# SolverForge/solverforge

Measured on AMD Instinct MI355X. Metric: moves-evaluated/sec, CVRP-1000 (nearby-list selector, LateAcceptance(400)+AcceptedCount(256)), higher is better.
Workload: dtype int64 score / int32 trial deltas (u16 matrix copy)

## Files before the change

solverforge_amd/_lib.py:

```python
import ctypes as C
import os

import numpy as np

_DIR = os.path.dirname(os.path.abspath(__file__))
LIB_PATH = os.environ.get("SF_AMD_LIB") or os.path.join(_DIR, "libsolverforge_amd.so")

SF_OK = 0
ERRORS = {-1: "SF_ERR_INVALID", -2: "SF_ERR_NO_DEVICE", -3: "SF_ERR_HIP", -4: "SF_ERR_UNSUPPORTED", -5: "SF_ERR_CAPACITY"}

MOVE_DTYPE = np.dtype(
    [("kind", "<i4"), ("a", "<i4"), ("a_pos", "<i4"), ("b", "<i4"), ("b_pos", "<i4"), ("value", "<i4")]
)
ANNEAL_CHUNK_DTYPE = np.dtype([("cur", "<i8", (4,)), ("sc", "<i8", (64, 4)), ("doable", "<u8"), ("nconsumed", "<i4"), ("step_end", "<i4")])
ANNEAL_STATE_WORDS = 32
ACCEPTOR_RECORD_DTYPE = np.dtype([("cur", "<i8", (4,)), ("sc", "<i8", (64, 4)), ("doable", "<u8"), ("op", "<i4"), ("reserved", "<i4")])
ACCEPTOR_STATE_WORDS = 9
TABU_SIGNATURE_DTYPE = np.dtype([("entity", "<u4", (2,)), ("value", "<u4", (2,)), ("move_id", "<u8", (2,)), ("undo_move_id", "<u8", (2,))])
TABU_RECORD_DTYPE = np.dtype([("score", "<i8", (4,)), ("sc", "<i8", (64, 4)), ("sig", TABU_SIGNATURE_DTYPE, (64,)), ("reach", "<u8"), ("op", "<i4"), ("has_sig", "<i4")])
TABU_STATE_FIXED = 16
TABU_MAX_TENURE_MOVE = 64
TABU_NO_TOKEN = 0xFFFFFFFF


# ... 166 lines not shown
    L.sf_portfolio_allgather_best.argtypes = [vp, vp, vp, vp]
    L.sf_portfolio_destroy.argtypes = [vp]
    L.sf_portfolio_broadcast_best.argtypes = [vp, i32, i32, vp, vp]
    L.sf_portfolio_migrate_local.argtypes = [vp, i32, i32, C.POINTER(i32)]
    L.sf_trace_digest_init.argtypes = [C.POINTER(TraceDigestStruct)]
    L.sf_trace_digest_update.argtypes = [C.POINTER(TraceDigestStruct), vp, C.c_size_t]
    L.sf_trace_encode_step.argtypes = [C.POINTER(TraceScopeStruct), u64, u64, vp, vp, i64, vp, i64, C.POINTER(TraceDigestStruct)]
    for name in SYMBOLS:
        fn = getattr(L, name)
        if name in ("sf_trace_digest_init", "sf_trace_digest_update"):
            fn.restype = None
        elif name == "sf_trace_encode_step":
            fn.restype = i64
        elif name not in ("sf_ctx_destroy", "sf_last_error"):
            fn.restype = i32
    _lib = L
    return L


def ptr(a):
    return a.ctypes.data_as(C.c_void_p) if a is not None else None


def check(rc, ctx=None):
    if rc == SF_OK:
        return
    msg = load().sf_last_error(ctx)
    raise SolverForgeError(f"{ERRORS.get(rc, rc)}: {msg.decode() if msg else ''}")
```

solverforge_amd/csrc/sf_api.hip:

```cpp
#include <hip/hip_runtime.h>

#include <algorithm>
#include <chrono>
#include <cmath>
#include <cstddef>
#include <cstdio>
#include <cstdlib>
#include <cstring>
#include <map>
#include <string>
#include <vector>

#define SF_TU_MAIN 1
#include "../../include/solverforge_amd.h"
#include "sf_launch.h"
#include "sf_construct.hip"
#include "sf_clarke_wright.hip"
#include "sf_kopt_tw.hip"
#include "sf_precedence.hip"
#include "sf_scalar_construct.h"

using namespace sf;

static std::string g_create_error;

struct Fact {
    int type = 0;
    void* d0 = nullptr;
    void* d1 = nullptr;
    int rows = 0, cols = 0;
    int64_t max_finite = 0;
    bool symmetric = false;
    bool all_finite = false;
    int64_t abs_sum = 0;
};
struct ConstraintSpec {
    int kind, desc, var, fact;
    int64_t param;
    int level;
    int64_t weight;
    std::vector<sf_pair_term> terms;
    std::vector<sf_uni_term> uterms;
    sf_uni_weight uweight{0, -1, -1, -1};
// ... 45 lines not shown
    std::map<int, ClassSpec> classes;
    std::map<int, Fact> facts;
    std::vector<ConstraintSpec> constraints;
    std::vector<SelectorSpec> selectors;
    bool initialized = false;
    bool has_list_model = false;
    int list_desc = -1;
    ListModel lm{};
    NearbyScalarSource nearby_scalar[2];
    int nearby_scalar_dynamic = 0;
    struct TwSpec {
        bool set = false, uploaded = false, force_walk = false, gate_ok = false;
        int desc = -1, n = 0;
        std::vector<int64_t> lo, hi, service, travel;
        int64_t departure = 0;
        int64_t *d_lo = nullptr, *d_hi = nullptr, *d_service = nullptr, *d_travel = nullptr;
        int32_t* d_ran = nullptr;
    } tw;
    PrecSpec prec;
    PrecModel pm{};
    bool prec_policy = false;
    PlfModel plf{};
    NbrIndex nbr{nullptr};
    ListModel lm_wave{};
    NbrIndex nbr_wave{nullptr};
    bool wave_renumbered = false;
    int last_wave_mode = -1;
    int32_t wave_spec_state = 0, wave_spec_reason = 0, wave_spec_key[18] = {};
    int n_cus = 0;
    int32_t last_generic_flags = -1;
    int32_t last_scalar_value_bytes = 0;
    int xown_level = -1;
    int64_t xown_weight = 0;
    std::vector<UniComponent> uni_components;
    uint16_t* d_xown_tab = nullptr;
    int64_t* d_xown_delta = nullptr;
    std::vector<std::pair<int, std::string>> providers;
    uint32_t* d_node_tab32 = nullptr;
    struct WaveFix {
        const uint16_t *perm, *inv, *mat16;
        const int32_t* demand;
        int32_t depot;
    } lm_wave_fix{};
    bool lm_small = false;
    int engine = SF_ENGINE_AUTO;
    bool has_scalar_model = false;
    int scalar_desc = -1;
    ScalarModel sm{};
    sf_solver_config cfg{SF_ACCEPT_LATE_ACCEPTANCE, 400, SF_FORAGER_ACCEPTED_COUNT, 256, 1, SF_ORDER_RANDOM, 0};
    SearchParams sp{};
    bool search_alloc = false;
// ... 843 lines not shown
        if (m.cap_level >= 0)
            ok = ok && dem < lim && mag(m.capacity) < lim && mag(m.cap_weight) < lim &&
                 mag(m.cap_weight) * 2 * (dem + mag(m.capacity) + 1) < ((int64_t)1 << 29);
        {
            static const bool off = std::getenv("SF_AMD_NO_SMALL") != nullptr;
            if (off) ok = false;
        }
        ctx->lm_small = ok;
        m.small32 = ok ? 1 : 0;
    }
    bool nearby = false;
    for (auto& s : ctx->selectors)
        if ((s.kind == SF_SEL_NEARBY_LIST_CHANGE || s.kind == SF_SEL_NEARBY_LIST_SWAP) && s.desc == d) nearby = true;
    int P = 2;
    while (P < m.dim) P <<= 1;
    if (nearby && m.mat && (size_t)P * 8 <= 128 * 1024) {
        uint16_t* keys = nullptr;
        if ((rc = dalloc(ctx, &keys, (size_t)m.dim * m.dim))) return rc;
        HIPCHK(ctx, hipFuncSetAttribute((const void*)k_nbr_presort, hipFuncAttributeMaxDynamicSharedMemorySize, P * 8));
        hipLaunchKernelGGL(k_nbr_presort, dim3(m.dim), dim3(256), (size_t)P * 8, ctx->stream, m.mat, m.dim, P, keys);
        HIPCHK(ctx, hipGetLastError());
        HIPCHK(ctx, hipStreamSynchronize(ctx->stream));
        ctx->nbr = NbrIndex{keys};
    }
    ctx->wave_renumbered = false;
    {
        const char* env = std::getenv("SF_AMD_RENUMBER");
        const bool want = env ? std::atoi(env) != 0 : (size_t)m.dim * m.dim * 2 > (size_t)1024 * 1024;
        if (want && ctx->nbr.keys && m.mat16 && ctx->lm_small && m.dim <= 0x7FFF && m.depot >= 0 && m.depot < m.dim) {
            const int dim = m.dim;
            std::vector<uint16_t> hk((size_t)dim * dim);
            HIPCHK(ctx, hipMemcpyAsync(hk.data(), ctx->nbr.keys, hk.size() * 2, hipMemcpyDeviceToHost, ctx->stream));
            HIPCHK(ctx, hipStreamSynchronize(ctx->stream));
            std::vector<uint16_t> perm((size_t)dim), inv((size_t)dim);
            std::vector<uint8_t> seen((size_t)dim, 0);
            std::vector<int> ptr((size_t)dim, 0);
            int cur = m.depot, low = 0;
            for (int n = 0; n < dim; ++n) {
                perm[(size_t)cur] = (uint16_t)n;
                inv[(size_t)n] = (uint16_t)cur;
                seen[(size_t)cur] = 1;
                if (n + 1 == dim) break;
                int nx = -1;
                const uint16_t* row = hk.data() + (size_t)cur * dim;
                for (int& t = ptr[(size_t)cur]; t < dim; ++t) {
                    const uint32_t e = row[t];
// ... 140 lines not shown
static int launch_list_wave(sf_ctx* ctx, const SearchParams& p, int n_replicas, bool trace) {
    WaveShape s = wave_shape(ctx);
    s.acceptor = p.acceptor, s.forager = p.forager, s.order = p.order, s.dry_run = p.dry_run, s.n_leaves = p.n_leaves;
    for (int l = 0; l < p.n_leaves && l < MAX_LEAVES; ++l) s.kind[l] = p.leaf[l].kind;
    s.n_replicas = n_replicas, s.trace = trace;
    const WavePlan pl = plan_wave_launch(s, wave_knobs());
    if (pl.err) return fail(ctx, pl.err, pl.msg);
    if (pl.nodeg && !ctx->lm.node_tab)
        if (int rc = dalloc(ctx, &ctx->lm.node_tab, (size_t)ctx->R * ctx->lm.dim)) return rc;
    SearchParams q = p;
    q.n_launch = n_replicas;
    SearchLaunch la = make_launch(ctx, &q, pl.grid, pl.block, (size_t)pl.lds);
    ctx->last_wave_mode = pl.mode;
    if (pl.compact && ctx->wave_renumbered) {
        ctx->lm_wave = ctx->lm;
        ctx->lm_wave.perm = ctx->lm_wave_fix.perm, ctx->lm_wave.inv = ctx->lm_wave_fix.inv, ctx->lm_wave.mat16 = ctx->lm_wave_fix.mat16;
        if (ctx->lm.demand) ctx->lm_wave.demand = ctx->lm_wave_fix.demand;
        ctx->lm_wave.depot = ctx->lm_wave_fix.depot;
        la.lm = &ctx->lm_wave;
        la.nb = ctx->nbr_wave;
    }
    if (!ctx->n_cus) HIPCHK(ctx, hipDeviceGetAttribute(&ctx->n_cus, hipDeviceAttributeMultiprocessorCount, ctx->device));
    const WaveSpecGate gate{pl.mode, q.move_budget != 0, (int32_t)std::min<int64_t>(std::max<int64_t>(q.n_steps, 0), INT32_MAX), n_replicas, pl.resident, ctx->n_cus, wave_spec_knob()};
    const WaveSpecKey key = wave_spec_key(pl.levels, pl.wpe, *la.lm, q, wave_spec_extras());
    ctx->wave_spec_state = SF_WSPEC_AOT, ctx->wave_spec_reason = wave_spec_wanted(gate);
    std::memcpy(ctx->wave_spec_key, &key, sizeof key);
    if (ctx->wave_spec_reason == SF_WSPEC_R_NONE) {
        hipFunction_t fn = nullptr;
        if ((ctx->wave_spec_reason = wave_spec_get(key, ctx->device, la.lds, &fn)) == SF_WSPEC_R_NONE) {
            WaveArgs args{*la.lm, q, la.nb};
            size_t n_args = sizeof args;
            void* cfg[] = {HIP_LAUNCH_PARAM_BUFFER_POINTER, &args, HIP_LAUNCH_PARAM_BUFFER_SIZE, &n_args, HIP_LAUNCH_PARAM_END};
            HIPCHK(ctx, hipModuleLaunchKernel(fn, (unsigned)la.grid, 1, 1, (unsigned)la.block, 1, 1, (unsigned)la.lds, la.stream, nullptr, cfg));
            ctx->wave_spec_state = SF_WSPEC_SPECIALISED;
            return SF_OK;
        }
        ctx->wave_spec_state = SF_WSPEC_FELL_BACK;
    }
    HIPCHK(ctx, pl.levels == 2 ? launch_tu_list_wave<2>(trace, pl.mode, la) : launch_tu_list_wave<4>(trace, pl.mode, la));
    return SF_OK;
}
static int launch_list_search(sf_ctx* ctx, const SearchParams& p, int grid, bool trace) {
    if (use_wave_engine(ctx)) return launch_list_wave(ctx, p, grid, trace);
    if (p.acceptor == SF_ACCEPT_DIVERSIFIED_LATE_ACCEPTANCE) return fail(ctx, SF_ERR_UNSUPPORTED, "DiversifiedLateAcceptance: wave, scalar and generic engines only");
    if (ctx->levels <= 2) return launch_list_search_t<2>(ctx, p, grid, trace);
    return launch_list_search_t<4>(ctx, p, grid, trace);
}
// ... 981 lines not shown
    std::memcpy(&k, knobs, sizeof k);
    if (s.n_leaves < 0 || s.n_leaves > GL) return SF_ERR_INVALID;
    const GenericPlan pl = plan_generic_launch(s, k);
    std::memcpy(plan, &pl, plan_bytes);
    if (msg) *msg = pl.msg;
    return pl.err;
}
extern "C" int32_t sf_debug_wave_plan(const int32_t* shape, int32_t n_shape, const int32_t* knobs, int32_t n_knobs, int32_t* plan, int32_t n_plan, const char** msg, int32_t* fits) {
    constexpr size_t plan_bytes = offsetof(WavePlan, msg);
    if (!shape || !knobs || !plan || n_shape * 4 != (int)sizeof(WaveShape) || n_knobs * 4 != (int)sizeof(WaveKnobs) || n_plan * 4 != (int)plan_bytes)
        return SF_ERR_INVALID;
    WaveShape s;
    WaveKnobs k;
    std::memcpy(&s, shape, sizeof s);
    std::memcpy(&k, knobs, sizeof k);
    const WavePlan pl = plan_wave_launch(s, k);
    std::memcpy(plan, &pl, plan_bytes);
    if (msg) *msg = pl.msg;
    if (fits) fits[0] = wave_engine_fits(s), fits[1] = wave_engine_default(s);
    return pl.err;
}

extern "C" int32_t sf_debug_wave_spec(const sf_ctx* ctx, int32_t* out, int32_t n_out) {
    if (!out || n_out != 4 + (int)(sizeof(WaveSpecKey) / 4)) return SF_ERR_INVALID;
    std::memset(out, 0, (size_t)n_out * 4);
    if (ctx) out[0] = ctx->wave_spec_state, out[1] = ctx->wave_spec_reason, std::memcpy(out + 4, ctx->wave_spec_key, sizeof(WaveSpecKey));
    WaveSpecCache& c = wave_spec_cache();
    std::lock_guard<std::mutex> lock(c.mu);
    out[2] = c.compiles, out[3] = (int32_t)std::ceil(c.last_ms);
    return SF_OK;
}
extern "C" int32_t sf_debug_late_acceptance(sf_ctx* ctx, int32_t replica, int64_t* out, int32_t n_slots, int32_t* cursor) {
    if (!ctx || !out || !cursor || !ctx->search_alloc || replica < 0 || replica >= ctx->R || n_slots != ctx->sp.la_size) return SF_ERR_INVALID;
    DeviceGuard guard(ctx);
    HIPCHK(ctx, hipStreamSynchronize(ctx->stream));
    HIPCHK(ctx, hipMemcpy(out, ctx->sp.la_hist + (size_t)replica * n_slots * 4, (size_t)n_slots * 32, hipMemcpyDeviceToHost));
    HIPCHK(ctx, hipMemcpy(cursor, ctx->sp.la_idx + replica, 4, hipMemcpyDeviceToHost));
    return SF_OK;
}
extern "C" int32_t sf_debug_wave_spec_gate(const int32_t* gate, int32_t n_gate) {
    if (!gate || n_gate * 4 != (int)sizeof(WaveSpecGate)) return SF_ERR_INVALID;
    WaveSpecGate g;
    std::memcpy(&g, gate, sizeof g);
    return wave_spec_wanted(g);
}
extern "C" int32_t sf_debug_wave_spec_compile(const int32_t* key, int32_t n_key, const char* arch, const char* out_path, char* opts, int32_t n_opts, char* log, int32_t n_log, double* ms) {
    if (!key || n_key * 4 != (int)sizeof(WaveSpecKey) || !arch) return SF_ERR_INVALID;
    WaveSpecKey k;
    std::memcpy(&k, key, sizeof k);
    if (!wave_spec_key_ok(k)) return SF_ERR_INVALID;
    const std::string csrc = wave_spec_csrc();
    auto put = [](char* dst, int32_t n, const std::string& s) {
        if (dst && n > 0) std::snprintf(dst, (size_t)n, "%s", s.c_str());
    };
    std::string o;
    for (auto& x : wave_spec_options(k, arch, csrc, wave_spec_rtc().include_dir)) o += x + "\n";
    put(opts, n_opts, o);
    if (!out_path) return SF_WSPEC_R_NONE;
    const WaveSpecBuild b = wave_spec_compile(k, arch, csrc);
    put(log, n_log, b.log);
    if (ms) *ms = b.ms;
    if (!b.reason) {
        std::ofstream f(out_path, std::ios::binary);
        f.write(b.code.data(), (std::streamsize)b.code.size());
        if (!f) return SF_ERR_INVALID;
    }
    return b.reason;
}

extern "C" int32_t sf_debug_step_arith(int32_t what, uint32_t start, uint32_t stride, uint32_t V, const uint32_t* k, int64_t n_k, uint32_t* out) {
    if (!k || !out || n_k < 0 || V < 2 || V > 1022 || (what != 0 && what != 1)) return SF_ERR_INVALID;
    const uint32_t rc = (uint32_t)(0x100000000ull / V);
// ... 31 lines not shown
```

solverforge_amd/csrc/sf_list_wave.hip:

```cpp
#pragma once
#include <hip/hip_runtime.h>
#include <stdint.h>

#include <type_traits>

#include "sf_list_model.h"

namespace sf {

constexpr uint32_t RC_MAX = 128;
constexpr uint32_t RC_SMALL = 64;
constexpr uint32_t NBR_NODE_MASK = 0x7FFFu;
constexpr uint32_t NBR_SAME_FLAG = 0x8000u;
constexpr uint32_t NBR_END = 0xFFFFu;
#ifndef SF_WPB
#define SF_WPB 4
#endif
constexpr int WPB = SF_WPB;

#ifndef SF_SPEC_V
#define SF_SPEC_V(x) (x)
#endif
#ifndef SF_SPEC_DIM
#define SF_SPEC_DIM(x) (x)
// ... 3 lines not shown
#endif
#ifndef SF_SPEC_K0
#define SF_SPEC_K0(x) (x)
#endif
#ifndef SF_SPEC_K1
#define SF_SPEC_K1(x) (x)
#endif
#ifndef SF_SPEC_LA_SIZE
#define SF_SPEC_LA_SIZE(x) (x)
#endif
#ifndef SF_SPEC_LIMIT
#define SF_SPEC_LIMIT(x) (x)
#endif
#ifndef SF_SPEC_HAS_PERM
#define SF_SPEC_HAS_PERM(x) (x)
#endif
#ifndef SF_SPEC_HAS_EXPLICIT
#define SF_SPEC_HAS_EXPLICIT(x) (x)
#endif
#ifdef SF_SPEC_L
#define SF_SPEC_OWN_LANE(v) asm volatile("" : "+v"(v))
#else
#define SF_SPEC_OWN_LANE(v)
#endif


__device__ __forceinline__ void wave_sync() {
    __builtin_amdgcn_fence(__ATOMIC_RELEASE, "wavefront");
    __builtin_amdgcn_wave_barrier();
    __builtin_amdgcn_fence(__ATOMIC_ACQUIRE, "wavefront");
}

SF_PLAIN_KERNEL
__global__ __launch_bounds__(256) void k_nbr_presort(const int64_t* __restrict__ mat, int dim, int P,
                                                     uint16_t* __restrict__ keys) {
    extern __shared__ __attribute__((aligned(16))) unsigned char smem[];
    uint64_t* sk = (uint64_t*)smem;
    const int row = blockIdx.x;
    const int64_t* rp = mat + (size_t)row * dim;
    for (int t = threadIdx.x; t < P; t += blockDim.x) {
        uint64_t k = ~0ULL;
        if (t < dim) {
            const int64_t v = rp[t];
            if (v >= 0 && v != UNREACHABLE) k = ((uint64_t)v << 24) | (uint64_t)(uint32_t)t;
        }
        sk[t] = k;
// ... 123 lines not shown
        const bool v0 = !intra || (dp != sp && dp != sp + 1);
        const bool v1 = dp + 1 == len2 && (!intra || len != sp + 1);
        it.w = some ? (uint32_t)v0 + (uint32_t)v1 : 0u;
        it.ord = intra ? (v0 ? dp : len) : inter_ord;
        it.pay0 = v0 ? slot : end_pay;
        it.pay1 = end_pay;
    } else {
        const bool v = intra ? dp > sp : rk > k;
        it.w = (some && v) ? 1u : 0u;
        it.ord = intra ? dp : inter_ord;
        it.pay0 = slot;
        it.pay1 = 0;
    }
    return it;
}

struct RouteTab {
    const uint32_t* rt;
    static constexpr int KEY_SHIFT = 24;
    __device__ __forceinline__ uint32_t word(uint32_t route) const { return rt[route]; }
    __device__ __forceinline__ static uint32_t rank(uint32_t w) { return w & 0xFFFFu; }
    __device__ __forceinline__ static uint32_t inter_ord(uint32_t w, uint32_t dp) { return ORD_INTER_BASE + (w >> 16) + dp; }
};
constexpr uint32_t ORD_ARITH_BASE = 1u << 26;
struct RouteArith {
    uint32_t st, inv, V, recip;
    static constexpr int KEY_SHIFT = 28;
    __device__ __forceinline__ uint32_t word(uint32_t route) const {
        uint32_t x = route + V - st;
        x = x >= V ? x - V : x;
        const uint32_t y = x * inv;
        uint32_t rk = y - __umulhi(y, recip) * V;
        return rk >= V ? rk - V : rk;
    }
    __device__ __forceinline__ static uint32_t rank(uint32_t w) { return w; }
    __device__ __forceinline__ static uint32_t inter_ord(uint32_t w, uint32_t dp) { return ORD_ARITH_BASE + (w << 16) + dp; }
};
struct RouteRank {
    const uint32_t* rt;
    static constexpr int KEY_SHIFT = RouteArith::KEY_SHIFT;
    __device__ __forceinline__ uint32_t word(uint32_t route) const { return rt[route]; }
    __device__ __forceinline__ static uint32_t rank(uint32_t w) { return w; }
    __device__ __forceinline__ static uint32_t inter_ord(uint32_t w, uint32_t dp) { return RouteArith::inter_ord(w, dp); }
};
template <class OT, class RT>
__device__ __forceinline__ NearbyItem nearby_item_rt(bool is_change, uint32_t slot, uint32_t se, uint32_t sp,
                                                     uint32_t len, uint32_t k, const OT* s_off, const RT& rt) {
    const bool some = slot != NODE_NONE;
    const uint32_t r2 = some ? slot >> 16 : 0u, dp = slot & 0xFFFFu;
    const uint32_t len2 = s_off[r2 + 1] - s_off[r2];
    const uint32_t t = rt.word(r2);
    const uint32_t rk = RT::rank(t);
    const uint32_t inter_ord = RT::inter_ord(t, dp);
    const bool intra = r2 == se;
    const uint32_t end_pay = (r2 << 16) | len2;
    NearbyItem it;
    if (is_change) {
        const bool v0 = !intra || (dp != sp && dp != sp + 1);
        const bool v1 = dp + 1 == len2 && (!intra || len != sp + 1);
        it.w = some ? (uint32_t)v0 + (uint32_t)v1 : 0u;
        it.ord = intra ? (v0 ? dp : len) : inter_ord;
        it.pay0 = v0 ? slot : end_pay;
        it.pay1 = end_pay;
    } else {
        const bool v = intra ? dp > sp : rk > k;
        it.w = (some && v) ? 1u : 0u;
        it.ord = intra ? dp : inter_ord;
        it.pay0 = slot;
        it.pay1 = 0;
    }
    return it;
}

__device__ __forceinline__ uint32_t mbcnt64(uint64_t mask) {
    return __builtin_amdgcn_mbcnt_hi((uint32_t)(mask >> 32), __builtin_amdgcn_mbcnt_lo((uint32_t)mask, 0u));
}

template <class LT, class OT, bool OWN_LANE = false>
__device__ __forceinline__ void apply_list_move_wave(const ListModel& m, uint16_t* visits, OT* off,
                                                     LT* load, int kind, uint32_t a, uint32_t i, uint32_t b,
                                                     uint32_t j, uint32_t ext = 0) {
    uint32_t lane = threadIdx.x & 63u;
    if constexpr (OWN_LANE) asm volatile("" : "+v"(lane));
    if (kind == 2) {
        const uint32_t P = off[a] + i, Q = off[b] + j;
        const uint32_t x = visits[P];
        wave_sync();
        if (P < Q) {
            for (uint32_t t0 = P; t0 < Q; t0 += 64) {
                const uint32_t t = t0 + lane;
                uint32_t nv = 0;
                if (t < Q) nv = (t + 1 < Q) ? (uint32_t)visits[t + 1] : x;
                wave_sync();
                if (t < Q) visits[t] = (uint16_t)nv;
                wave_sync();
            }
        } else if (P > Q) {
            for (uint32_t c0 = 0; c0 <= P - Q; c0 += 64) {
                const uint32_t dd = c0 + lane;
// ... 782 lines not shown
        }
        ISA_MARK("prologue_end");

        PH(1)
        int done = 0;
        while (!done) {
            PH(4)
            auto gen_rest = [&](int l, uint32_t se, uint32_t sp, uint32_t len, uint32_t k, uint32_t sx, uint32_t tl,
                                uint32_t key, uint32_t base, uint32_t need, uint32_t emitted) -> uint32_t {
                const bool is_change = l ? chg1 : chg0;
                const RT rt = route_facts(l);
                uint32_t* rq = ring + (size_t)l * cv.rc * 2;
                const uint16_t* rowk = nb.keys + (size_t)sx * dim;
                const uint32_t mv0 = (se << 16) | sp;
                for (;;) {
                    const bool have = key != NBR_END;
                    const uint64_t havemask = __ballot(have);
                    if (havemask == 0) break;
                    NearbyItem it{0u, 0u, 0u, 0u};
                    if (have) it = nearby_item_rt(is_change, node_slot.get(key & NBR_NODE_MASK), se, sp, len, k, s_off, rt);
                    const uint64_t startmask = __ballot(have && (lane == 0 || !(key & NBR_SAME_FLAG)));
                    const bool more = havemask == ~0ULL && base + 64 < dim;
                    const uint32_t fo = 63u - (uint32_t)__clzll((unsigned long long)startmask);
                    if (more && fo == 0) {
                        TopK tk{~0ULL, 0u, ~0ULL};
                        for (uint32_t b2 = base; b2 < dim; b2 += 64) {
                            const uint32_t j2 = b2 + lane;
                            const uint32_t ky = j2 < dim ? (uint32_t)rowk[j2] : NBR_END;
                            NearbyItem i2{0u, 0u, 0u, 0u};
                            uint64_t hk = 0;
                            if (ky != NBR_END) {
                                const uint32_t y2 = ky & NBR_NODE_MASK;
                                i2 = nearby_item_rt(is_change, node_slot.get(y2), se, sp, len, k, s_off, rt);
                                hk = (uint64_t)m.mat[(size_t)ext_id(sx) * dim + ext_id(y2)] << RT::KEY_SHIFT;
                            }
                            if (!__ballot(ky != NBR_END)) break;
                            topk_offer(tk, need, i2.w >= 1 ? (hk | i2.ord) : ~0ULL, i2.pay0);
                            topk_offer(tk, need, i2.w == 2 ? (hk | (i2.ord + 1)) : ~0ULL, i2.pay1);
                        }
                        const uint32_t cnt = (uint32_t)__popcll(__ballot(lane < need && tk.key != ~0ULL));
                        if (lane < cnt) {
                            const uint32_t qi = (tl + emitted + lane) & RCM;
                            rq[qi * 2] = mv0;
                            rq[qi * 2 + 1] = tk.pay;
                        }
                        emitted += cnt;
                        break;
                    }
                    const uint32_t nclosed = more ? fo : (uint32_t)__popcll(havemask);
                    const uint64_t closedmask = nclosed >= 64 ? ~0ULL : ((1ULL << nclosed) - 1ULL);
                    const bool closed = (closedmask & lanebit) != 0;
                    const uint32_t wc = closed ? it.w : 0u;
                    const uint64_t w1 = __ballot(wc == 1), w2 = __ballot(wc == 2);
                    const uint32_t Wc = (uint32_t)__popcll(w1) + 2u * (uint32_t)__popcll(w2);
                    GC(l ? 6 : 5)
                    if (Wc == 0) { GC(7) }
                    if (Wc > 0) {
                        int32_t pos = (int32_t)(mbcnt64(w1) + 2u * mbcnt64(w2));
                        const uint64_t nonstart = ~startmask & closedmask;
                        if (nonstart) {
                            const uint32_t packed = (it.ord << 2) | wc;
                            uint64_t run = nonstart;
                            uint32_t p_dn = packed, p_up = packed;
                            for (uint32_t d = 1; run != 0; ++d) {
                                p_dn = (uint32_t)__builtin_amdgcn_update_dpp(0, (int)p_dn, 0x130, 0xf, 0xf, false);
                                p_up = (uint32_t)__builtin_amdgcn_update_dpp(0, (int)p_up, 0x138, 0xf, 0xf, false);
                                const bool same_up = (run & lanebit) != 0;
                                const bool same_dn = ((run >> d) & lanebit) != 0;
                                if (same_dn && (p_dn >> 2) < it.ord) pos += (int32_t)(p_dn & 3u);
                                if (same_up && (p_up >> 2) > it.ord) pos -= (int32_t)(p_up & 3u);
                                run &= nonstart << d;
                            }
                        }
                        if (wc >= 1 && (uint32_t)pos < need) {
                            const uint32_t qi = (tl + emitted + (uint32_t)pos) & RCM;
                            rq[qi * 2] = mv0;
                            rq[qi * 2 + 1] = it.pay0;
                        }
                        if (wc == 2 && (uint32_t)pos + 1 < need) {
                            const uint32_t qi = (tl + emitted + (uint32_t)pos + 1) & RCM;
                            rq[qi * 2] = mv0;
                            rq[qi * 2 + 1] = it.pay1;
                        }
                        const uint32_t ne = Wc < need ? Wc : need;
                        emitted += ne;
                        need -= ne;
                    }
                    if (need == 0 || !more) break;
                    base += nclosed;
                    const uint32_t jj = base + lane;
                    key = jj < dim ? (uint32_t)rowk[jj] : NBR_END;
                }
                return emitted;
            };
            auto slot_of = [&](uint32_t word, uint32_t node) -> uint32_t {
                if constexpr (SAT) {
                    uint32_t ns = nsat;
                    asm volatile("" : "+s"(ns));
                    if (ns != 0) return node_slot.wide(word, node);
                    return node_slot.wide_short(word);
                } else
                    return node_slot.wide(word, node);
            };
            const uint32_t single0 = cv.rc - K0 < 64u ? cv.rc - K0 : 64u, single1 = cv.rc - K1 < 64u ? cv.rc - K1 : 64u;
            ISA_MARK("fill_begin");
            for (;;) {
                const bool both_live = !C0.ex && !C1.ex;
                const bool need0 = !C0.ex && C0.left > 0 && C0.tail - C0.head < (both_live ? 32u : single0);
                const bool need1 = n_leaves > 1 && !C1.ex && C1.left > 0 && C1.tail - C1.head < (both_live ? 32u : single1);
                if (!need0 && !need1) break;
                if (need0 && need1) {
                    ISA_MARK("pair_begin");
                    GC(0)
                    const bool hi = lane >= 32;
                    const uint32_t seA = C0.se, spA = C0.sp, lenA = C0.len, kA = C0.k, sxA = C0.sx, tlA = C0.tail;
                    const uint32_t seB = C1.se, spB = C1.sp, lenB = C1.len, kB = C1.k, sxB = C1.sx, tlB = C1.tail;
                    uint32_t l31 = lane & 31u;
                    if constexpr (LEAN) asm volatile("" : "+v"(l31));
                    const uint32_t key = LEAN ? row_key(half(C0.pk, C1.pk), l31) : (hi ? C1.pk : C0.pk);
                    const bool have = key != NBR_END;
                    uint32_t nd = have ? (key & NBR_NODE_MASK) : 0u;
                    uint32_t slot_word = 0;
                    if constexpr (LEAN) {
                        asm volatile("" : "+v"(nd)::"memory");
                        slot_word = node_slot.word(nd);
                    }
                    C0.left -= 1;
                    C0.o += 1;
                    if (C0.left > 0) resolve(C0, 0);
                    C1.left -= 1;
                    C1.o += 1;
                    if (C1.left > 0) resolve(C1, 1);
                    if constexpr (!SMALL) st_sources += 2;
                    uint32_t slot_any;
                    if constexpr (LEAN)
                        slot_any = slot_of(slot_word, nd);
                    else
                        slot_any = node_slot.get(nd);
                    const uint32_t slot = have ? slot_any : NODE_NONE;
                    NearbyItem it{0u, 0u, 0u, 0u};
                    uint32_t mv0, tl, Kh, rq_off;
                    if constexpr (LEAN) {
                        const uint32_t sev = half(seA, seB), spv = half(spA, spB);
// ... 42 lines not shown
                        if constexpr (FAST) {
                            const bool some = slot != NODE_NONE;
                            const uint32_t r2 = some ? slot >> 16 : 0u, dp = slot & 0xFFFFu;
                            const uint32_t len2 = s_off[r2 + 1] - s_off[r2];
                            const uint32_t t = rth.word(r2);
                            const bool intra = r2 == se;
                            const uint32_t end_pay = (r2 << 16) | len2;
                            const bool v0 = hi ? (intra ? dp > sp : RT::rank(t) > kk) : (!intra || dp - sp >= 2u);
                            const bool v1 = !hi && dp + 1 == len2 && (!intra || len != sp + 1);
                            it.w = some ? (uint32_t)v0 + (uint32_t)v1 : 0u;
                            it.ord = intra ? ((hi || v0) ? dp : len) : RT::inter_ord(t, dp);
                            it.pay0 = (hi || v0) ? slot : end_pay;
                            it.pay1 = end_pay;
                        } else {
                            const NearbyItem ic = nearby_item_rt(true, slot, se, sp, len, kk, s_off, rth);
                            const NearbyItem is = nearby_item_rt(false, slot, se, sp, len, kk, s_off, rth);
                            const bool lane_change = hi ? chg1 : chg0;
                            it.w = lane_change ? ic.w : is.w;
                            it.ord = lane_change ? ic.ord : is.ord;
                            it.pay0 = lane_change ? ic.pay0 : is.pay0;
                            it.pay1 = lane_change ? ic.pay1 : is.pay1;
                        }
                    }
                    const uint64_t havemask = __ballot(have);
                    const uint64_t startmask = LEAN ? __ballot(key < NBR_END - min(l31, 1u) * (NBR_END - NBR_SAME_FLAG))
                                                        : __ballot(have && (l31 == 0 || !(key & NBR_SAME_FLAG)));
                    const uint32_t hvA = (uint32_t)havemask, hvB = (uint32_t)(havemask >> 32);
                    const uint32_t stA = (uint32_t)startmask, stB = (uint32_t)(startmask >> 32);
                    const bool moreA = hvA == 0xFFFFFFFFu && 32u < dim, moreB = hvB == 0xFFFFFFFFu && 32u < dim;
                    uint32_t ncA = 0, ncB = 0;
                    uint64_t closedmask;
                    bool closed;
                    if constexpr (LEAN) {
                        const uint32_t hvv = half(hvA, hvB), stv = half(stA, stB);
                        const uint32_t ncv = (hvv == 0xFFFFFFFFu && 32u < dim) ? 31u - (uint32_t)__clz(stv) : (uint32_t)__popc(hvv);
                        closed = l31 < ncv;
                        closedmask = __ballot(closed);
                    } else {
                        ncA = moreA ? 31u - (uint32_t)__clz(stA) : (uint32_t)__popc(hvA);
                        ncB = moreB ? 31u - (uint32_t)__clz(stB) : (uint32_t)__popc(hvB);
                        closedmask = (uint64_t)(ncA >= 32 ? 0xFFFFFFFFu : ((1u << ncA) - 1u)) |
                                     ((uint64_t)(ncB >= 32 ? 0xFFFFFFFFu : ((1u << ncB) - 1u)) << 32);
                        closed = (closedmask & lanebit) != 0;
                    }
                    const uint32_t wc = closed ? it.w : 0u;
                    const uint64_t w1 = __ballot(wc == 1), w2 = __ballot(wc == 2);
                    const uint32_t WcA = (uint32_t)__popc((uint32_t)w1) + 2u * (uint32_t)__popc((uint32_t)w2);
                    const uint32_t WcB = (uint32_t)__popc((uint32_t)(w1 >> 32)) + 2u * (uint32_t)__popc((uint32_t)(w2 >> 32));
                    if (WcA + WcB > 0) {
                        const uint32_t pa = __builtin_amdgcn_mbcnt_lo((uint32_t)w1, 0u) + 2u * __builtin_amdgcn_mbcnt_lo((uint32_t)w2, 0u);
                        const uint32_t pb = __builtin_amdgcn_mbcnt_hi((uint32_t)(w1 >> 32), 0u) + 2u * __builtin_amdgcn_mbcnt_hi((uint32_t)(w2 >> 32), 0u);
                        int32_t pos = (int32_t)(LEAN ? half(pa, pb) : (hi ? pb : pa));
                        const uint64_t nonstart = ~startmask & closedmask;
                        if (nonstart) {
                            const uint32_t packed = (it.ord << 2) | wc;
                            uint64_t run = nonstart;
                            uint32_t p_dn = packed, p_up = packed;
                            for (uint32_t d = 1; run != 0; ++d) {
                                p_dn = (uint32_t)__builtin_amdgcn_update_dpp(0, (int)p_dn, 0x130, 0xf, 0xf, false);
                                p_up = (uint32_t)__builtin_amdgcn_update_dpp(0, (int)p_up, 0x138, 0xf, 0xf, false);
                                const bool same_up = (run & lanebit) != 0;
                                const bool same_dn = ((run >> d) & lanebit) != 0;
                                if (same_dn && (p_dn >> 2) < it.ord) pos += (int32_t)(p_dn & 3u);
                                if (same_up && (p_up >> 2) > it.ord) pos -= (int32_t)(p_up & 3u);
                                run &= nonstart << d;
                            }
                        }
                        uint32_t* rq = ring + rq_off;
                        if (wc >= 1 && (uint32_t)pos < Kh) {
                            const uint32_t qi = (tl + (uint32_t)pos) & RCM;
                            rq[qi * 2] = mv0;
                            rq[qi * 2 + 1] = it.pay0;
                        }
                        if (wc == 2 && (uint32_t)pos + 1 < Kh) {
                            const uint32_t qi = (tl + (uint32_t)pos + 1) & RCM;
                            rq[qi * 2] = mv0;
                            rq[qi * 2 + 1] = it.pay1;
                        }
                    }
                    uint32_t emA = WcA < K0 ? WcA : K0, emB = WcB < K1 ? WcB : K1;
                    if (emA < K0 && moreA) {
                        GC(3)
                        ISA_MARK("pair_rest_begin");
                        if constexpr (LEAN) ncA = 31u - (uint32_t)__clz(stA);
                        const uint32_t jj = ncA + lane;
                        emA = gen_rest(0, seA, spA, lenA, kA, sxA, tlA, jj < dim ? (uint32_t)nb.keys[(size_t)sxA * dim + jj] : NBR_END, ncA, K0 - emA, emA);
                        ISA_MARK("pair_rest_end");
                    }
                    if (emB < K1 && moreB) {
                        GC(4)
// ... 481 lines not shown
```

solverforge_amd/csrc/sf_wave_spec.h:

```cpp
#pragma once
#include <dlfcn.h>

#include <fstream>
#include <mutex>
#include <sstream>

struct WaveSpecKey {
    int32_t levels, wpe;
    int32_t V, dim, n_cap, k0, k1;
    int32_t extras;
    int32_t capacity, cap_weight, dist_weight, depot, cap_level, dist_level;
    int32_t la_size, limit, has_perm, has_explicit;
};
enum { SF_WSPEC_X_MODEL = 1, SF_WSPEC_X_LA = 2, SF_WSPEC_X_LIMIT = 4, SF_WSPEC_X_PERM = 8, SF_WSPEC_X_EXPLICIT = 16, SF_WSPEC_X_ALL = 31 };
constexpr int32_t SF_WSPEC_X_DEFAULT = SF_WSPEC_X_MODEL | SF_WSPEC_X_LA | SF_WSPEC_X_PERM;
static int32_t wave_spec_extras() {
    const char* e = std::getenv("SF_AMD_WAVE_SPEC_EXTRAS");
    return e ? (std::atoi(e) & SF_WSPEC_X_ALL) : SF_WSPEC_X_DEFAULT;
}
template <class Model, class Params>
static WaveSpecKey wave_spec_key(int32_t levels, int32_t wpe, const Model& m, const Params& q, int32_t extras) {
    WaveSpecKey k{};
    k.levels = levels, k.wpe = wpe, k.V = m.V, k.dim = m.dim, k.n_cap = m.n_cap, k.k0 = q.leaf[0].max_nearby, k.k1 = q.leaf[1].max_nearby;
    auto fits = [](int64_t v) { return v >= INT32_MIN && v <= INT32_MAX; };
    if ((extras & SF_WSPEC_X_MODEL) && !(fits(m.capacity) && fits(m.cap_weight) && fits(m.dist_weight))) extras &= ~SF_WSPEC_X_MODEL;
    if ((m.perm != nullptr) != (m.inv != nullptr)) extras &= ~SF_WSPEC_X_PERM;
    k.extras = extras;
    if (extras & SF_WSPEC_X_MODEL)
        k.capacity = (int32_t)m.capacity, k.cap_weight = (int32_t)m.cap_weight, k.dist_weight = (int32_t)m.dist_weight, k.depot = m.depot, k.cap_level = m.cap_level,
        k.dist_level = m.dist_level;
    if (extras & SF_WSPEC_X_LA) k.la_size = q.la_size;
    if (extras & SF_WSPEC_X_LIMIT) k.limit = q.limit;
    if (extras & SF_WSPEC_X_PERM) k.has_perm = m.perm != nullptr && m.inv != nullptr;
    if (extras & SF_WSPEC_X_EXPLICIT) k.has_explicit = q.explicit_seeds != nullptr;
    return k;
}
struct WaveSpecGate {
    int32_t mode, move_budget, n_steps;
    int32_t n_replicas, resident, cus;
    int32_t knob;
};
enum {
    SF_WSPEC_AOT = 0, SF_WSPEC_SPECIALISED = 1, SF_WSPEC_FELL_BACK = 2,
    SF_WSPEC_R_NONE = 0,
    SF_WSPEC_R_KNOB = 1, SF_WSPEC_R_MODE = 2, SF_WSPEC_R_BUDGET = 3, SF_WSPEC_R_STEPS = 4, SF_WSPEC_R_RESIDENCY = 5,
    SF_WSPEC_R_NO_HIPRTC = 10, SF_WSPEC_R_NO_SOURCES = 11, SF_WSPEC_R_COMPILE = 12, SF_WSPEC_R_LOAD = 13, SF_WSPEC_R_LDS = 14,
// ... 15 lines not shown
}

static std::vector<std::string> wave_spec_options(const WaveSpecKey& k, const std::string& arch, const std::string& csrc, const std::string& rocm_include) {
    auto def = [](const char* name, int32_t v) { return std::string("-D") + name + "(x)=" + std::to_string(v); };
    std::vector<std::string> o{"--offload-arch=" + arch, "-O3", "-std=c++17", "-ffp-contract=off"};
    o.push_back("-I" + csrc);
    if (!rocm_include.empty()) o.push_back("-I" + rocm_include);
    o.push_back("-DSF_SPEC_L=" + std::to_string(k.levels));
    o.push_back("-DSF_SPEC_WPE=" + std::to_string(k.wpe));
    o.push_back(def("SF_SPEC_V", k.V));
    o.push_back(def("SF_SPEC_DIM", k.dim));
    o.push_back(def("SF_SPEC_NCAP", k.n_cap));
    o.push_back(def("SF_SPEC_K0", k.k0));
    o.push_back(def("SF_SPEC_K1", k.k1));
    auto word = [](const char* name, int32_t v) { return std::string("-D") + name + "=(" + std::to_string(v) + ")"; };
    if (k.extras & SF_WSPEC_X_MODEL)
        for (auto& x : {word("SF_SPEC_MODEL_WORDS", 1), word("SF_SPEC_CAPACITY", k.capacity), word("SF_SPEC_CAP_WEIGHT", k.cap_weight), word("SF_SPEC_DIST_WEIGHT", k.dist_weight),
                        word("SF_SPEC_DEPOT", k.depot), word("SF_SPEC_CAP_LEVEL", k.cap_level), word("SF_SPEC_DIST_LEVEL", k.dist_level)})
            o.push_back(x);
    if (k.extras & SF_WSPEC_X_LA) o.push_back(def("SF_SPEC_LA_SIZE", k.la_size));
    if (k.extras & SF_WSPEC_X_LIMIT) o.push_back(def("SF_SPEC_LIMIT", k.limit));
    if (k.extras & SF_WSPEC_X_PERM) o.push_back(def("SF_SPEC_HAS_PERM", k.has_perm));
    if (k.extras & SF_WSPEC_X_EXPLICIT) o.push_back(def("SF_SPEC_HAS_EXPLICIT", k.has_explicit));
    return o;
}
static std::string wave_spec_kernel_expr(const WaveSpecKey& k) {
    return "sf::k_list_search_wave<" + std::to_string(k.levels) + ", false, 2, true, " + std::to_string(k.wpe) + ", false>";
}
static bool wave_spec_key_ok(const WaveSpecKey& k) {
    return (k.levels == 2 || k.levels == 4) && k.wpe >= 4 && k.wpe <= 6 && k.V >= 1 && k.dim >= 1 && k.n_cap >= 0 && k.k0 >= 1 && k.k1 >= 1 && (k.extras & ~SF_WSPEC_X_ALL) == 0 &&
           (!(k.extras & SF_WSPEC_X_LA) || k.la_size >= 1) && (!(k.extras & SF_WSPEC_X_LIMIT) || k.limit >= 1);
}

struct WaveSpecRtc {
    void* lib = nullptr;
    std::string include_dir;
    int (*create)(void**, const char*, const char*, int, const char**, const char**) = nullptr;
    int (*compile)(void*, int, const char**) = nullptr;
    int (*destroy)(void**) = nullptr;
    int (*add_name)(void*, const char*) = nullptr;
    int (*lowered)(void*, const char*, const char**) = nullptr;
    int (*code_size)(void*, size_t*) = nullptr;
    int (*code)(void*, char*) = nullptr;
    int (*log_size)(void*, size_t*) = nullptr;
    int (*log)(void*, char*) = nullptr;
    bool ok() const { return lib && create && compile && destroy && add_name && lowered && code_size && code && log_size && log; }
};
static std::string wave_spec_dirname(const std::string& p) {
    const size_t s = p.find_last_of('/');
    return s == std::string::npos ? std::string(".") : p.substr(0, s);
}
static const WaveSpecRtc& wave_spec_rtc() {
    static const WaveSpecRtc once = [] {
        WaveSpecRtc r;
// ... 125 lines not shown
```

Measured before the change: 71.87 billion.

## Specialize wave kernel on neighbor-index facts: tie runs, full rows, packed tie key

Scans the presorted neighbor key table on the host once at setup to find the longest tie run and whether every row has at least 64 finite entries. These facts go into the runtime-compiled wave kernel key as macros. The macros drop the wide-tie fallback loop, drop tie fixups when there are no ties, make the have/havemask ballots constant for full rows, and use a compact packed tie-order key that needs fewer bits. This removes branches and ballots from the hot neighbor-scan loop, at the cost of a host scan at setup and more specialization variants to compile.

```diff
diff --git a/solverforge_amd/_lib.py b/solverforge_amd/_lib.py
--- a/solverforge_amd/_lib.py
+++ b/solverforge_amd/_lib.py
@@ -212,6 +212,15 @@
     return a.ctypes.data_as(C.c_void_p) if a is not None else None
 
 
+def nbr_facts(keys):
+    a = np.ascontiguousarray(keys, dtype=np.uint16)
+    out = (C.c_int32 * 2)()
+    fn = C.CDLL(LIB_PATH).sf_debug_nbr_facts
+    fn.restype = C.c_int32
+    check(fn(ptr(a), a.shape[0], a.shape[1], out, 2))
+    return int(out[0]), int(out[1])
+
+
 def check(rc, ctx=None):
     if rc == SF_OK:
         return
diff --git a/solverforge_amd/csrc/sf_api.hip b/solverforge_amd/csrc/sf_api.hip
--- a/solverforge_amd/csrc/sf_api.hip
+++ b/solverforge_amd/csrc/sf_api.hip
@@ -19,6 +19,7 @@
 #include "sf_kopt_tw.hip"
 #include "sf_precedence.hip"
 #include "sf_scalar_construct.h"
+#include "sf_nbr_facts.h"
 
 using namespace sf;
 
@@ -110,11 +111,12 @@
     bool prec_policy = false;
     PlfModel plf{};
     NbrIndex nbr{nullptr};
+    NbrFacts nbr_facts{};
     ListModel lm_wave{};
     NbrIndex nbr_wave{nullptr};
     bool wave_renumbered = false;
     int last_wave_mode = -1;
-    int32_t wave_spec_state = 0, wave_spec_reason = 0, wave_spec_key[18] = {};
+    int32_t wave_spec_state = 0, wave_spec_reason = 0, wave_spec_key[22] = {};
     int n_cus = 0;
     int32_t last_generic_flags = -1;
     int32_t last_scalar_value_bytes = 0;
@@ -1004,6 +1006,16 @@
         HIPCHK(ctx, hipGetLastError());
         HIPCHK(ctx, hipStreamSynchronize(ctx->stream));
         ctx->nbr = NbrIndex{keys};
+        NbrFacts nf{0, 1};
+        const int64_t rows_per = std::max<int64_t>(1, ((int64_t)4 << 20) / m.dim);
+        std::vector<uint16_t> part((size_t)std::min<int64_t>(rows_per, m.dim) * m.dim);
+        for (int64_t r0 = 0; r0 < m.dim; r0 += rows_per) {
+            const int64_t n = std::min<int64_t>(rows_per, m.dim - r0);
+            HIPCHK(ctx, hipMemcpyAsync(part.data(), keys + (size_t)r0 * m.dim, (size_t)n * m.dim * 2, hipMemcpyDeviceToHost, ctx->stream));
+            HIPCHK(ctx, hipStreamSynchronize(ctx->stream));
+            nbr_facts_rows(part.data(), n, m.dim, nf);
+        }
+        ctx->nbr_facts = nf;
     }
     ctx->wave_renumbered = false;
     {
@@ -1190,7 +1202,7 @@
     }
     if (!ctx->n_cus) HIPCHK(ctx, hipDeviceGetAttribute(&ctx->n_cus, hipDeviceAttributeMultiprocessorCount, ctx->device));
     const WaveSpecGate gate{pl.mode, q.move_budget != 0, (int32_t)std::min<int64_t>(std::max<int64_t>(q.n_steps, 0), INT32_MAX), n_replicas, pl.resident, ctx->n_cus, wave_spec_knob()};
-    const WaveSpecKey key = wave_spec_key(pl.levels, pl.wpe, *la.lm, q, wave_spec_extras());
+    const WaveSpecKey key = wave_spec_key(pl.levels, pl.wpe, *la.lm, q, ctx->nbr_facts, wave_spec_extras());
     ctx->wave_spec_state = SF_WSPEC_AOT, ctx->wave_spec_reason = wave_spec_wanted(gate);
     std::memcpy(ctx->wave_spec_key, &key, sizeof key);
     if (ctx->wave_spec_reason == SF_WSPEC_R_NONE) {
@@ -2218,9 +2230,10 @@
 }
 
 extern "C" int32_t sf_debug_wave_spec(const sf_ctx* ctx, int32_t* out, int32_t n_out) {
-    if (!out || n_out != 4 + (int)(sizeof(WaveSpecKey) / 4)) return SF_ERR_INVALID;
+    static_assert(sizeof(WaveSpecKey) == sizeof(sf_ctx::wave_spec_key), "WaveSpecKey");
+    if (!out || (n_out != 4 + (int)(sizeof(WaveSpecKey) / 4) && n_out != 4 + SF_WSPEC_KEY_WORDS_V1)) return SF_ERR_INVALID;
     std::memset(out, 0, (size_t)n_out * 4);
-    if (ctx) out[0] = ctx->wave_spec_state, out[1] = ctx->wave_spec_reason, std::memcpy(out + 4, ctx->wave_spec_key, sizeof(WaveSpecKey));
+    if (ctx) out[0] = ctx->wave_spec_state, out[1] = ctx->wave_spec_reason, std::memcpy(out + 4, ctx->wave_spec_key, (size_t)(n_out - 4) * 4);
     WaveSpecCache& c = wave_spec_cache();
     std::lock_guard<std::mutex> lock(c.mu);
     out[2] = c.compiles, out[3] = (int32_t)std::ceil(c.last_ms);
@@ -2240,10 +2253,21 @@
     std::memcpy(&g, gate, sizeof g);
     return wave_spec_wanted(g);
 }
+extern "C" int32_t sf_debug_nbr_facts(const uint16_t* keys, int32_t rows, int32_t dim, int32_t* out, int32_t n_out) {
+    if (!keys || !out || rows < 1 || dim < 1 || n_out != 2) return SF_ERR_INVALID;
+    NbrFacts f{0, 1};
+    nbr_facts_rows(keys, rows, dim, f);
+    out[0] = f.tie_max, out[1] = f.rows_full;
+    return SF_OK;
+}
+extern "C" int32_t sf_debug_wave_spec_index_gate(const int32_t* in, int32_t n_in) {
+    if (!in || n_in != 5 || in[0] < 1 || in[1] < 1 || in[2] < 0) return SF_ERR_INVALID;
+    return wave_spec_index_allowed(WaveSpecIndexGate{in[0], in[1], in[2], in[3] >= 64, in[3] >= 2, in[4] != 0});
+}
 extern "C" int32_t sf_debug_wave_spec_compile(const int32_t* key, int32_t n_key, const char* arch, const char* out_path, char* opts, int32_t n_opts, char* log, int32_t n_log, double* ms) {
-    if (!key || n_key * 4 != (int)sizeof(WaveSpecKey) || !arch) return SF_ERR_INVALID;
-    WaveSpecKey k;
-    std::memcpy(&k, key, sizeof k);
+    if (!key || (n_key * 4 != (int)sizeof(WaveSpecKey) && n_key != SF_WSPEC_KEY_WORDS_V1) || !arch) return SF_ERR_INVALID;
+    WaveSpecKey k{};
+    std::memcpy(&k, key, (size_t)n_key * 4);
     if (!wave_spec_key_ok(k)) return SF_ERR_INVALID;
     const std::string csrc = wave_spec_csrc();
     auto put = [](char* dst, int32_t n, const std::string& s) {
diff --git a/solverforge_amd/csrc/sf_list_wave.hip b/solverforge_amd/csrc/sf_list_wave.hip
--- a/solverforge_amd/csrc/sf_list_wave.hip
+++ b/solverforge_amd/csrc/sf_list_wave.hip
@@ -49,6 +49,23 @@
 #define SF_SPEC_OWN_LANE(v) asm volatile("" : "+v"(v))
 #else
 #define SF_SPEC_OWN_LANE(v)
+#endif
+#ifdef SF_SPEC_NO_WIDE
+#define SF_SPEC_WIDE_TIES(x) false
+#else
+#define SF_SPEC_WIDE_TIES(x) (x)
+#endif
+#ifdef SF_SPEC_NO_TIES
+#define SF_SPEC_TIES(x) 0ULL
+#else
+#define SF_SPEC_TIES(x) (x)
+#endif
+#ifdef SF_SPEC_ROWS_FULL
+#define SF_SPEC_ROW_HAVE(x) true
+#define SF_SPEC_ROW_HAVEMASK(x) (~0ULL)
+#else
+#define SF_SPEC_ROW_HAVE(x) (x)
+#define SF_SPEC_ROW_HAVEMASK(x) (x)
 #endif
 
 
@@ -218,7 +235,14 @@
     __device__ __forceinline__ static uint32_t rank(uint32_t w) { return w & 0xFFFFu; }
     __device__ __forceinline__ static uint32_t inter_ord(uint32_t w, uint32_t dp) { return ORD_INTER_BASE + (w >> 16) + dp; }
 };
+#ifdef SF_SPEC_TIE_KEY
+static_assert(SF_SPEC_RB >= 1 && SF_SPEC_PB >= 1 && SF_SPEC_RB + SF_SPEC_PB <= 22, "SF_SPEC_TIE_KEY: the packed word does not fit 32 bits");
+constexpr uint32_t ORD_ARITH_BASE = 1u << (SF_SPEC_RB + SF_SPEC_PB);
+constexpr int ORD_ARITH_SHIFT = SF_SPEC_PB;
+#else
 constexpr uint32_t ORD_ARITH_BASE = 1u << 26;
+constexpr int ORD_ARITH_SHIFT = 16;
+#endif
 struct RouteArith {
     uint32_t st, inv, V, recip;
     static constexpr int KEY_SHIFT = 28;
@@ -230,7 +254,7 @@
         return rk >= V ? rk - V : rk;
     }
     __device__ __forceinline__ static uint32_t rank(uint32_t w) { return w; }
-    __device__ __forceinline__ static uint32_t inter_ord(uint32_t w, uint32_t dp) { return ORD_ARITH_BASE + (w << 16) + dp; }
+    __device__ __forceinline__ static uint32_t inter_ord(uint32_t w, uint32_t dp) { return ORD_ARITH_BASE + (w << ORD_ARITH_SHIFT) + dp; }
 };
 struct RouteRank {
     const uint32_t* rt;
@@ -271,6 +295,22 @@
 __device__ __forceinline__ uint32_t mbcnt64(uint64_t mask) {
     return __builtin_amdgcn_mbcnt_hi((uint32_t)(mask >> 32), __builtin_amdgcn_mbcnt_lo((uint32_t)mask, 0u));
 }
+#ifdef SF_SPEC_TIE_KEY
+__device__ __forceinline__ int32_t tie_key_fix(uint64_t startmask, uint64_t nonstart, uint32_t ord, uint32_t wc) {
+    const uint32_t q = (mbcnt64(startmask >> 1) << (SF_SPEC_RB + SF_SPEC_PB + 3)) | (ord << 2) | wc;
+    uint32_t q_dn = q, q_up = q;
+    int32_t fix = 0;
+    uint64_t run = nonstart;
+    for (uint32_t d = 1; run != 0; ++d) {
+        q_dn = (uint32_t)__builtin_amdgcn_update_dpp(0, (int)q_dn, 0x130, 0xf, 0xf, true);
+        q_up = (uint32_t)__builtin_amdgcn_update_dpp(0, (int)q_up, 0x138, 0xf, 0xf, true);
+        fix += q_dn < q ? (int32_t)(q_dn & 3u) : 0;
+        fix -= q_up > q ? (int32_t)(q_up & 3u) : 0;
+        run &= nonstart << d;
+    }
+    return fix;
+}
+#endif
 
 template <class LT, class OT, bool OWN_LANE = false>
 __device__ __forceinline__ void apply_list_move_wave(const ListModel& m, uint16_t* visits, OT* off,
@@ -1099,7 +1139,7 @@
                     const uint64_t startmask = __ballot(have && (lane == 0 || !(key & NBR_SAME_FLAG)));
                     const bool more = havemask == ~0ULL && base + 64 < dim;
                     const uint32_t fo = 63u - (uint32_t)__clzll((unsigned long long)startmask);
-                    if (more && fo == 0) {
+                    if (SF_SPEC_WIDE_TIES(more && fo == 0)) {
                         TopK tk{~0ULL, 0u, ~0ULL};
                         for (uint32_t b2 = base; b2 < dim; b2 += 64) {
                             const uint32_t j2 = b2 + lane;
@@ -1134,7 +1174,10 @@
                     if (Wc == 0) { GC(7) }
                     if (Wc > 0) {
                         int32_t pos = (int32_t)(mbcnt64(w1) + 2u * mbcnt64(w2));
-                        const uint64_t nonstart = ~startmask & closedmask;
+                        const uint64_t nonstart = SF_SPEC_TIES(~startmask & closedmask);
+#ifdef SF_SPEC_TIE_KEY
+                        if (nonstart) pos += tie_key_fix(startmask, nonstart, it.ord, wc);
+#else
                         if (nonstart) {
                             const uint32_t packed = (it.ord << 2) | wc;
                             uint64_t run = nonstart;
@@ -1149,6 +1192,7 @@
                                 run &= nonstart << d;
                             }
                         }
+#endif
                         if (wc >= 1 && (uint32_t)pos < need) {
                             const uint32_t qi = (tl + emitted + (uint32_t)pos) & RCM;
                             rq[qi * 2] = mv0;
@@ -1194,8 +1238,8 @@
                     const uint32_t seB = C1.se, spB = C1.sp, lenB = C1.len, kB = C1.k, sxB = C1.sx, tlB = C1.tail;
                     uint32_t l31 = lane & 31u;
                     if constexpr (LEAN) asm volatile("" : "+v"(l31));
-                    const uint32_t key = LEAN ? row_key(half(C0.pk, C1.pk), l31) : (hi ? C1.pk : C0.pk);
-                    const bool have = key != NBR_END;
+                    const uint32_t key = LEAN ? (SF_SPEC_ROW_HAVE(false) ? half(C0.pk, C1.pk) : row_key(half(C0.pk, C1.pk), l31)) : (hi ? C1.pk : C0.pk);
+                    const bool have = SF_SPEC_ROW_HAVE(key != NBR_END);
                     uint32_t nd = have ? (key & NBR_NODE_MASK) : 0u;
                     uint32_t slot_word = 0;
                     if constexpr (LEAN) {
@@ -1284,7 +1328,7 @@
                             it.pay1 = lane_change ? ic.pay1 : is.pay1;
                         }
                     }
-                    const uint64_t havemask = __ballot(have);
+                    const uint64_t havemask = SF_SPEC_ROW_HAVEMASK(__ballot(have));
                     const uint64_t startmask = LEAN ? __ballot(key < NBR_END - min(l31, 1u) * (NBR_END - NBR_SAME_FLAG))
                                                         : __ballot(have && (l31 == 0 || !(key & NBR_SAME_FLAG)));
                     const uint32_t hvA = (uint32_t)havemask, hvB = (uint32_t)(havemask >> 32);
@@ -1313,7 +1357,11 @@
                         const uint32_t pa = __builtin_amdgcn_mbcnt_lo((uint32_t)w1, 0u) + 2u * __builtin_amdgcn_mbcnt_lo((uint32_t)w2, 0u);
                         const uint32_t pb = __builtin_amdgcn_mbcnt_hi((uint32_t)(w1 >> 32), 0u) + 2u * __builtin_amdgcn_mbcnt_hi((uint32_t)(w2 >> 32), 0u);
                         int32_t pos = (int32_t)(LEAN ? half(pa, pb) : (hi ? pb : pa));
-                        const uint64_t nonstart = ~startmask & closedmask;
+                        const uint64_t nonstart = SF_SPEC_TIES(~startmask & closedmask);
+#ifdef SF_SPEC_TIE_KEY
+                        static_assert(!std::is_same<RT, RouteTab>::value, "SF_SPEC_TIE_KEY: the (rank, position) ordinals");
+                        if (nonstart) pos += tie_key_fix(startmask, nonstart, it.ord, wc);
+#else
                         if (nonstart) {
                             const uint32_t packed = (it.ord << 2) | wc;
                             uint64_t run = nonstart;
@@ -1328,6 +1376,7 @@
                                 run &= nonstart << d;
                             }
                         }
+#endif
                         uint32_t* rq = ring + rq_off;
                         if (wc >= 1 && (uint32_t)pos < Kh) {
                             const uint32_t qi = (tl + (uint32_t)pos) & RCM;
diff --git a/solverforge_amd/csrc/sf_nbr_facts.h b/solverforge_amd/csrc/sf_nbr_facts.h
--- /dev/null
+++ b/solverforge_amd/csrc/sf_nbr_facts.h
@@ -0,0 +1,20 @@
+#pragma once
+#include <stdint.h>
+
+struct NbrFacts {
+    int32_t tie_max = 64;
+    int32_t rows_full = 0;
+};
+static inline void nbr_facts_rows(const uint16_t* keys, int64_t rows, int32_t dim, NbrFacts& f) {
+    const int32_t full = dim < 64 ? dim : 64;
+    for (int64_t r = 0; r < rows; ++r) {
+        const uint16_t* row = keys + r * dim;
+        int32_t finite = 0, run = 0;
+        for (int32_t t = 0; t < dim && row[t] != 0xFFFFu; ++t) {
+            ++finite;
+            run = (t > 0 && (row[t] & 0x8000u)) ? run + 1 : 1;
+            if (run > f.tie_max) f.tie_max = run < 64 ? run : 64;
+        }
+        if (finite < full) f.rows_full = 0;
+    }
+}
diff --git a/solverforge_amd/csrc/sf_wave_spec.h b/solverforge_amd/csrc/sf_wave_spec.h
--- a/solverforge_amd/csrc/sf_wave_spec.h
+++ b/solverforge_amd/csrc/sf_wave_spec.h
@@ -1,5 +1,7 @@
 #pragma once
 #include <dlfcn.h>
+
+#include "sf_nbr_facts.h"
 
 #include <fstream>
 #include <mutex>
@@ -11,17 +13,45 @@
     int32_t extras;
     int32_t capacity, cap_weight, dist_weight, depot, cap_level, dist_level;
     int32_t la_size, limit, has_perm, has_explicit;
-};
+    int32_t wide_ties, ties, rows_full;
+    int32_t index_x;
+};
+constexpr int32_t SF_WSPEC_KEY_WORDS_V1 = 18;
 enum { SF_WSPEC_X_MODEL = 1, SF_WSPEC_X_LA = 2, SF_WSPEC_X_LIMIT = 4, SF_WSPEC_X_PERM = 8, SF_WSPEC_X_EXPLICIT = 16, SF_WSPEC_X_ALL = 31 };
+enum { SF_WSPEC_X_NO_WIDE = 32, SF_WSPEC_X_TIE_KEY = 64, SF_WSPEC_X_NO_TIES = 128, SF_WSPEC_X_ROWS_FULL = 256, SF_WSPEC_X_INDEX_ALL = 480 };
 constexpr int32_t SF_WSPEC_X_DEFAULT = SF_WSPEC_X_MODEL | SF_WSPEC_X_LA | SF_WSPEC_X_PERM;
+constexpr int32_t SF_WSPEC_X_INDEX_DEFAULT = SF_WSPEC_X_NO_WIDE | SF_WSPEC_X_TIE_KEY | SF_WSPEC_X_ROWS_FULL;
 static int32_t wave_spec_extras() {
     const char* e = std::getenv("SF_AMD_WAVE_SPEC_EXTRAS");
-    return e ? (std::atoi(e) & SF_WSPEC_X_ALL) : SF_WSPEC_X_DEFAULT;
+    return e ? (std::atoi(e) & (SF_WSPEC_X_ALL | SF_WSPEC_X_INDEX_ALL)) : (SF_WSPEC_X_DEFAULT | SF_WSPEC_X_INDEX_DEFAULT);
+}
+
+struct WaveSpecIndexGate {
+    int32_t V, dim, n_cap;
+    int32_t wide_ties, ties, rows_full;
+};
+static int32_t wave_spec_bits(uint32_t v) {
+    int32_t b = 1;
+    while (v >> b) ++b;
+    return b;
+}
+static int32_t wave_spec_rb(int32_t V) { return wave_spec_bits((uint32_t)(V > 1 ? V - 1 : 0)); }
+static int32_t wave_spec_pb(int32_t n_cap) { return wave_spec_bits((uint32_t)(n_cap > 0 ? n_cap : 0)); }
+static int32_t wave_spec_index_allowed(const WaveSpecIndexGate& g) {
+    int32_t a = 0;
+    if (!g.wide_ties) a |= SF_WSPEC_X_NO_WIDE;
+    if (wave_spec_rb(g.V) + wave_spec_pb(g.n_cap) <= 22) a |= SF_WSPEC_X_TIE_KEY;
+    if (!g.ties) a |= SF_WSPEC_X_NO_TIES;
+    if (g.rows_full && g.dim >= 32) a |= SF_WSPEC_X_ROWS_FULL;
+    return a;
 }
 template <class Model, class Params>
-static WaveSpecKey wave_spec_key(int32_t levels, int32_t wpe, const Model& m, const Params& q, int32_t extras) {
+static WaveSpecKey wave_spec_key(int32_t levels, int32_t wpe, const Model& m, const Params& q, const NbrFacts& nf, int32_t extras) {
     WaveSpecKey k{};
     k.levels = levels, k.wpe = wpe, k.V = m.V, k.dim = m.dim, k.n_cap = m.n_cap, k.k0 = q.leaf[0].max_nearby, k.k1 = q.leaf[1].max_nearby;
+    k.wide_ties = nf.tie_max >= 64, k.ties = nf.tie_max >= 2, k.rows_full = nf.rows_full != 0;
+    k.index_x = extras & SF_WSPEC_X_INDEX_ALL & wave_spec_index_allowed(WaveSpecIndexGate{k.V, k.dim, k.n_cap, k.wide_ties, k.ties, k.rows_full});
+    extras &= SF_WSPEC_X_ALL;
     auto fits = [](int64_t v) { return v >= INT32_MIN && v <= INT32_MAX; };
     if ((extras & SF_WSPEC_X_MODEL) && !(fits(m.capacity) && fits(m.cap_weight) && fits(m.dist_weight))) extras &= ~SF_WSPEC_X_MODEL;
     if ((m.perm != nullptr) != (m.inv != nullptr)) extras &= ~SF_WSPEC_X_PERM;
@@ -83,6 +113,11 @@
     if (k.extras & SF_WSPEC_X_LIMIT) o.push_back(def("SF_SPEC_LIMIT", k.limit));
     if (k.extras & SF_WSPEC_X_PERM) o.push_back(def("SF_SPEC_HAS_PERM", k.has_perm));
     if (k.extras & SF_WSPEC_X_EXPLICIT) o.push_back(def("SF_SPEC_HAS_EXPLICIT", k.has_explicit));
+    if (k.index_x & SF_WSPEC_X_NO_WIDE) o.push_back(word("SF_SPEC_NO_WIDE", 1));
+    if (k.index_x & SF_WSPEC_X_TIE_KEY)
+        for (auto& x : {word("SF_SPEC_TIE_KEY", 1), word("SF_SPEC_RB", wave_spec_rb(k.V)), word("SF_SPEC_PB", wave_spec_pb(k.n_cap))}) o.push_back(x);
+    if (k.index_x & SF_WSPEC_X_NO_TIES) o.push_back(word("SF_SPEC_NO_TIES", 1));
+    if (k.index_x & SF_WSPEC_X_ROWS_FULL) o.push_back(word("SF_SPEC_ROWS_FULL", 1));
     return o;
 }
 static std::string wave_spec_kernel_expr(const WaveSpecKey& k) {
@@ -90,7 +125,9 @@
 }
 static bool wave_spec_key_ok(const WaveSpecKey& k) {
     return (k.levels == 2 || k.levels == 4) && k.wpe >= 4 && k.wpe <= 6 && k.V >= 1 && k.dim >= 1 && k.n_cap >= 0 && k.k0 >= 1 && k.k1 >= 1 && (k.extras & ~SF_WSPEC_X_ALL) == 0 &&
-           (!(k.extras & SF_WSPEC_X_LA) || k.la_size >= 1) && (!(k.extras & SF_WSPEC_X_LIMIT) || k.limit >= 1);
+           (!(k.extras & SF_WSPEC_X_LA) || k.la_size >= 1) && (!(k.extras & SF_WSPEC_X_LIMIT) || k.limit >= 1) &&
+           (k.wide_ties | k.ties | k.rows_full | 1) == 1 && (!k.wide_ties || k.ties) &&
+           (k.index_x & ~wave_spec_index_allowed(WaveSpecIndexGate{k.V, k.dim, k.n_cap, k.wide_ties, k.ties, k.rows_full})) == 0;
 }
 
 struct WaveSpecRtc {
```

New measurement: 77.38 billion, median of 6. +7.7%, better.
